# tnibler/local-features

Measured on AMD Instinct MI355X. Metric: MKD descriptors/sec (32x32 patch, 128-D), higher is better.
Workload: dtype f32 (f16x3 split MFMA pooling)

## Files before the change

### local-features_amd/csrc/mkd_describe.hip

```cpp
#include <hip/hip_runtime.h>
#include <stdint.h>

#include <type_traits>

#include "mkd_ablate.h"
#include "mkd_device.h"
#include "mkd_sample.h"

namespace lfmkd {


namespace {

typedef _Float16 f16x8 __attribute__((ext_vector_type(8)));
typedef unsigned int u32x4 __attribute__((ext_vector_type(4)));
typedef float f32x2 __attribute__((ext_vector_type(2)));
__device__ __forceinline__ f32x2 pk_fma(f32x2 a, f32x2 b, f32x2 c) { return __builtin_elementwise_fma(a, b, c); }
__device__ __forceinline__ f32x2 pk_set(float v) { return f32x2{v, v}; }

__device__ __host__ constexpr bool f16_family(int pool) { return pool == LF_POOL_F16X3 || pool == LF_POOL_F16_FP6; }

__device__ __host__ constexpr bool fold_form(int pool) { return pool != LF_POOL_F16_FP6; }
constexpr int kTiles = 21;
constexpr int kAccTiles = 21, kUnfAccTiles = 24;
// ... 5 lines not shown

constexpr float kB0 = 0.0096f, kB1 = 0.2054f, kB2 = 0.5699f;

__device__ __host__ constexpr int row_bytes(bool fold) { return lut_pieces(fold) * 1024; }
__device__ __host__ constexpr int ring_off(bool fold) { return 2 * row_bytes(fold); }
constexpr int kRowBytes = row_bytes(true), kRingOff = ring_off(true);
constexpr int kRingSlots = 6;
[[maybe_unused]] constexpr int kSrcPatches = 0, kSrcKeypoints = 1, kSrcKeypointsSplit = 2;
constexpr int kRingSlotsKp = 12;
constexpr int kLevelTableBytes = 5 * kMaxPyrLevels * 4;

__device__ __forceinline__ float lane_fetch(int byte_addr, float v) {
    return __int_as_float(__builtin_amdgcn_ds_bpermute(byte_addr, __float_as_int(v)));
}

__device__ __forceinline__ void lds_dma16(const void *gsrc, void *ldst) {
    __builtin_amdgcn_global_load_lds((const __attribute__((address_space(1))) void *)gsrc,
                                     (__attribute__((address_space(3))) void *)ldst, 16, 0, 0);
}
__device__ __forceinline__ void lds_dma16_sv(const unsigned char *uniform_base, unsigned lane_off, void *ldst) {
    asm("" : "+s"(uniform_base));
    asm volatile("" : "+v"(lane_off));
    lds_dma16(uniform_base + lane_off, ldst);
}

template <int W, bool FOLD, bool ODDV>
__device__ __forceinline__ void issue_lut_row(const unsigned char *__restrict__ lut_rows, int row,
                                              unsigned char *lds_row, int wave, int lane) {
    static_assert(!ODDV || FOLD, "the folded forms' tiles");
    constexpr int kPieces = ODDV ? lut_pieces(FOLD) - 8 : lut_pieces(FOLD);
    const unsigned lane16 = (unsigned)lane * 16u;
#pragma unroll
    for (int j = 0; j < (kPieces + W - 1) / W; ++j) {
        if (wave + W * j < kPieces) {
            const int i = wave + W * j, piece = ODDV ? i + 2 * (i >> 2) : i;
            const unsigned char *g = lut_rows + ((size_t)row * row_bytes(FOLD) + (size_t)piece * 1024);
            lds_dma16_sv(g, lane16, lds_row + piece * 1024);
        }
    }
}

constexpr int kWStepBytes = 16384;
__device__ __forceinline__ constexpr int wstage_slot(int step) { return step % 3 == 0 ? 0 : (step % 3 == 1 ? 32768 : 16384); }
static_assert(wstage_slot(0) + kWStepBytes <= row_bytes(true) && wstage_slot(10) >= row_bytes(false) &&
              wstage_slot(10) + kWStepBytes <= 2 * row_bytes(true), "both forms' row buffers");

template <int W>
__device__ __forceinline__ void issue_w_step(const unsigned char *__restrict__ wfrag, int step, unsigned char *lds,
                                             int wave, int lane) {
    const unsigned lane16 = (unsigned)lane * 16u;
    unsigned char *d = lds + wstage_slot(step);
#pragma unroll
    for (int j = 0; j < 16 / W; ++j) {
        const unsigned char *g = wfrag + ((size_t)step * kWStepBytes + (size_t)(wave + W * j) * 1024);
        lds_dma16_sv(g, lane16, d + (wave + W * j) * 1024);
    }
}

template <int N> __device__ __forceinline__ void wait_vmcnt() { asm volatile("s_waitcnt vmcnt(%0)" ::"n"(N) : "memory"); }

struct RawSrc { const unsigned char *base; unsigned lane_off; };
__device__ __forceinline__ void issue_raw_row(const RawSrc &src, int row, unsigned char *ring, int slot) {
    const int y = row < 0 ? 0 : (row > 31 ? 31 : row);
    const unsigned char *g = src.base + y * 128;
    lds_dma16_sv(g, src.lane_off, ring + slot * 2048);
    lds_dma16_sv(g + 64, src.lane_off, ring + slot * 2048 + 1024);
}

#pragma clang fp contract(off)

__device__ __forceinline__ float max3_tiny(float a, float b) {
    return __builtin_fmaxf(__builtin_fmaxf(a, b), 1e-30f);
}

template <int ANGLE>
__device__ __forceinline__ void gradient_direction(f32x2 gx, f32x2 gy, f32x2 r2, f32x2 &ct, f32x2 &st) {
    if (ANGLE == LF_ANGLE_EXACT || ANGLE == LF_ANGLE_EXACT_ZERO) {
        const f32x2 inv = {__builtin_amdgcn_rsqf(r2.x), __builtin_amdgcn_rsqf(r2.y)};
        const f32x2 c = gx * inv, s = -gy * inv;
        const bool z0 = ANGLE == LF_ANGLE_EXACT ? r2.x == 0.f : gx.x == 0.f;
        const bool z1 = ANGLE == LF_ANGLE_EXACT ? r2.y == 0.f : gx.y == 0.f;
        ct = f32x2{z0 ? 1.f : c.x, z1 ? 1.f : c.y};
        st = f32x2{z0 ? 0.f : s.x, z1 ? 0.f : s.y};
    } else {
        const float ax0 = fabsf(gx.x), ay0 = fabsf(gy.x), ax1 = fabsf(gx.y), ay1 = fabsf(gy.y);
        const bool sw0 = ax0 < ay0 && gx.x != 0.f, sw1 = ax1 < ay1 && gx.y != 0.f;
        const f32x2 mn = {__builtin_fminf(ax0, ay0), __builtin_fminf(ax1, ay1)};
        const f32x2 mx = {max3_tiny(ax0, ay0), max3_tiny(ax1, ay1)};
        const f32x2 a = mn * f32x2{__builtin_amdgcn_rcpf(mx.x), __builtin_amdgcn_rcpf(mx.y)};
        const f32x2 s = a * a;
        f32x2 p = pk_fma(s, pk_set(-0.0117212f), pk_set(0.05265332f));
        p = pk_fma(s, p, pk_set(-0.11643287f));
        p = pk_fma(s, p, pk_set(0.19354346f));
        p = pk_fma(s, p, pk_set(-0.33262347f));
        p = pk_fma(s, p, pk_set(0.99997726f));
        p = a * p;
        const f32x2 p2 = p * p;
// ... 150 lines not shown
    }
};

template <int POOL, int PART>
__device__ __forceinline__ void mma_part(const AFrag<POOL> &a, const BFrag &b, f32x4 &acc) {
    static_assert(POOL == LF_POOL_F32 || POOL == LF_POOL_F16X3, "the three-term / f32 forms");
    if constexpr (ablate::kNoMma && POOL == LF_POOL_F16X3) {
        asm volatile("" ::"v"(a.hi), "v"(a.lo), "v"(b.p0), "v"(b.p1));
        return;
    }
    if constexpr (POOL == LF_POOL_F32) {
        const f32x4 b0 = __builtin_bit_cast(f32x4, b.p0), b1 = __builtin_bit_cast(f32x4, b.p1);
        if (PART == 0) {
#pragma unroll
            for (int e = 0; e < 3; ++e) acc = __builtin_amdgcn_mfma_f32_16x16x4f32(b0[e], a.v[e], acc, 0, 0, 0);
        } else if (PART == 1) {
            acc = __builtin_amdgcn_mfma_f32_16x16x4f32(b0[3], a.v[3], acc, 0, 0, 0);
            acc = __builtin_amdgcn_mfma_f32_16x16x4f32(b1[0], a.v[4], acc, 0, 0, 0);
            acc = __builtin_amdgcn_mfma_f32_16x16x4f32(b1[1], a.v[5], acc, 0, 0, 0);
        } else {
            acc = __builtin_amdgcn_mfma_f32_16x16x4f32(b1[2], a.v[6], acc, 0, 0, 0);
            acc = __builtin_amdgcn_mfma_f32_16x16x4f32(b1[3], a.v[7], acc, 0, 0, 0);
        }
    } else {
        const f16x8 bh = __builtin_bit_cast(f16x8, b.p0), bl = __builtin_bit_cast(f16x8, b.p1);
        const f16x8 ah = __builtin_bit_cast(f16x8, a.hi), al = __builtin_bit_cast(f16x8, a.lo);
        if (PART == 0) acc = __builtin_amdgcn_mfma_f32_16x16x32_f16(bh, al, acc, 0, 0, 0);
        else if (PART == 1) acc = __builtin_amdgcn_mfma_f32_16x16x32_f16(bl, ah, acc, 0, 0, 0);
        else acc = __builtin_amdgcn_mfma_f32_16x16x32_f16(bh, ah, acc, 0, 0, 0);
    }
}

template <class SlotOfTap>
__device__ __forceinline__ void blur_row_impl(const unsigned char *ring_lane, SlotOfTap slot_of_tap, int addr_l, int addr_r,
                                              bool has_l, bool has_r, float (&out)[8], float &out_l, float &out_r) {
    if constexpr (ablate::kNoFrontEnd) {
        const int sl = slot_of_tap(0);
        const f32x4 a_ = *reinterpret_cast<const f32x4 *>(ring_lane + sl * 2048);
        const f32x4 b_ = *reinterpret_cast<const f32x4 *>(ring_lane + sl * 2048 + 256);
#pragma unroll
        for (int x = 0; x < 4; ++x) { out[x] = a_[x]; out[4 + x] = b_[x]; }
        out_l = out[0];
        out_r = out[7];
        return;
    }
    float vb[8];
    {
        const float kk[5] = {kB0, kB1, kB2, kB1, kB0};
        f32x2 v2[4];
#pragma unroll
        for (int i = 0; i < 5; ++i) {
            const int sl = slot_of_tap(i);
            const f32x4 lo = *reinterpret_cast<const f32x4 *>(ring_lane + sl * 2048);
            const f32x4 hi = *reinterpret_cast<const f32x4 *>(ring_lane + sl * 2048 + 256);
            const f32x2 r[4] = {{lo[0], lo[1]}, {lo[2], lo[3]}, {hi[0], hi[1]}, {hi[2], hi[3]}};
#pragma unroll
            for (int e = 0; e < 4; ++e) v2[e] = i == 0 ? pk_set(kk[0]) * r[e] : pk_fma(pk_set(kk[i]), r[e], v2[e]);
        }
#pragma unroll
        for (int e = 0; e < 4; ++e) { vb[2 * e] = v2[e].x; vb[2 * e + 1] = v2[e].y; }
    }
    float ext[12];
    const float l0 = lane_fetch(addr_l, vb[6]), l1 = lane_fetch(addr_l, vb[7]);
    const float r0 = lane_fetch(addr_r, vb[0]), r1 = lane_fetch(addr_r, vb[1]);
    ext[0] = has_l ? l0 : vb[0];
    ext[1] = has_l ? l1 : vb[0];
    ext[10] = has_r ? r0 : vb[7];
    ext[11] = has_r ? r1 : vb[7];
#pragma unroll
    for (int x = 0; x < 8; ++x) ext[2 + x] = vb[x];
#pragma unroll
    for (int x = 0; x < 8; ++x) {
        float s = ablate::kMulFirstTap ? kB0 * ext[x] : fmaf(kB0, ext[x], 0.0f);
        s = fmaf(kB1, ext[x + 1], s);
        s = fmaf(kB2, ext[x + 2], s);
        s = fmaf(kB1, ext[x + 3], s);
        s = fmaf(kB0, ext[x + 4], s);
        out[x] = s;
    }
    const float hl = lane_fetch(addr_l, out[7]), hr = lane_fetch(addr_r, out[0]);
    out_l = has_l ? hl : out[0];
    out_r = has_r ? hr : out[7];
}

template <class SlotOfTap>
__device__ __forceinline__ void blur_row_fold_impl(const unsigned char *ring_a, const unsigned char *ring_b, SlotOfTap slot_of_tap,
                                                   int addr_l, int addr_r, bool has_l, bool has_r, float (&out)[8],
                                                   float (&nb)[4]) {
    if constexpr (ablate::kNoFrontEnd) {
        const int sl = slot_of_tap(0);
        const f32x4 a_ = *reinterpret_cast<const f32x4 *>(ring_a + sl * 2048);
        const f32x4 b_ = *reinterpret_cast<const f32x4 *>(ring_b + sl * 2048);
#pragma unroll
        for (int x = 0; x < 4; ++x) { out[x] = a_[x]; out[4 + x] = b_[3 - x]; }
        nb[0] = out[0]; nb[1] = out[3]; nb[2] = out[7]; nb[3] = out[4];
        return;
    }
    float va[4], vb[4];
    {
        const float kk[5] = {kB0, kB1, kB2, kB1, kB0};
        f32x2 v2[4];
#pragma unroll
        for (int i = 0; i < 5; ++i) {
            const int sl = slot_of_tap(i);
            const f32x4 lo = *reinterpret_cast<const f32x4 *>(ring_a + sl * 2048);
            const f32x4 hi = *reinterpret_cast<const f32x4 *>(ring_b + sl * 2048);
            const f32x2 r[4] = {{lo[0], lo[1]}, {lo[2], lo[3]}, {hi[0], hi[1]}, {hi[2], hi[3]}};
#pragma unroll
            for (int e = 0; e < 4; ++e) v2[e] = i == 0 ? pk_set(kk[0]) * r[e] : pk_fma(pk_set(kk[i]), r[e], v2[e]);
        }
        va[0] = v2[0].x; va[1] = v2[0].y; va[2] = v2[1].x; va[3] = v2[1].y;
        vb[0] = v2[2].x; vb[1] = v2[2].y; vb[2] = v2[3].x; vb[3] = v2[3].y;
    }
    float ea[8], eb[8];
    {
        const float la0 = lane_fetch(addr_l, va[2]), la1 = lane_fetch(addr_l, va[3]);
        const float rb0 = lane_fetch(addr_l, vb[0]), rb1 = lane_fetch(addr_l, vb[1]);
        const float ra0 = lane_fetch(addr_r, va[0]), ra1 = lane_fetch(addr_r, va[1]);
        const float lb0 = lane_fetch(addr_r, vb[2]), lb1 = lane_fetch(addr_r, vb[3]);
        ea[0] = has_l ? la0 : va[0];
        ea[1] = has_l ? la1 : va[0];
        ea[6] = has_r ? ra0 : vb[0];
        ea[7] = has_r ? ra1 : vb[1];
        eb[0] = has_r ? lb0 : va[2];
        eb[1] = has_r ? lb1 : va[3];
        eb[6] = has_l ? rb0 : vb[3];
        eb[7] = has_l ? rb1 : vb[3];
    }
#pragma unroll
    for (int x = 0; x < 4; ++x) { ea[2 + x] = va[x]; eb[2 + x] = vb[x]; }
    float ob[4];
#pragma unroll
    for (int x = 0; x < 4; ++x) {
        float s = ablate::kMulFirstTap ? kB0 * ea[x] : fmaf(kB0, ea[x], 0.0f);
        s = fmaf(kB1, ea[x + 1], s);
        s = fmaf(kB2, ea[x + 2], s);
        s = fmaf(kB1, ea[x + 3], s);
        s = fmaf(kB0, ea[x + 4], s);
        out[x] = s;
        float t = ablate::kMulFirstTap ? kB0 * eb[x] : fmaf(kB0, eb[x], 0.0f);
        t = fmaf(kB1, eb[x + 1], t);
        t = fmaf(kB2, eb[x + 2], t);
        t = fmaf(kB1, eb[x + 3], t);
        t = fmaf(kB0, eb[x + 4], t);
        ob[x] = t;
    }
#pragma unroll
    for (int x = 0; x < 4; ++x) out[4 + x] = ob[3 - x];
    const float hal = lane_fetch(addr_l, out[3]), hbr = lane_fetch(addr_l, ob[0]);
    const float har = lane_fetch(addr_r, out[0]), hbl = lane_fetch(addr_r, ob[3]);
    nb[0] = has_l ? hal : out[0];
    nb[1] = has_r ? har : ob[0];
    nb[2] = has_r ? hbl : out[3];
    nb[3] = has_l ? hbr : ob[3];
}

__device__ __forceinline__ void fold_sum(const f32x2 (&s)[4], f32x2 &e0, f32x2 &e1) { e0 = s[0] + s[2]; e1 = s[1] + s[3]; }
__device__ __forceinline__ void fold_diff(const f32x2 (&s)[4], f32x2 &o0, f32x2 &o1) { o0 = s[0] - s[2]; o1 = s[1] - s[3]; }
__device__ __forceinline__ void fold_diff_rev(const f32x2 (&s)[4], f32x2 &o0, f32x2 &o1) { o0 = s[2] - s[0]; o1 = s[3] - s[1]; }

__device__ __forceinline__ void odd_cart_row(const f32x2 (&fx)[2], const f32x4 &gy, f32x2 h0, f32x2 h1, float (&oc)[3]) {
    const f32x2 r = pk_fma(fx[1], h1, fx[0] * h0);
    const float t = r.x + r.y;
#pragma unroll
    for (int b = 0; b < 3; ++b) oc[b] = __builtin_fmaf(gy[b], t, oc[b]);
}

__device__ __forceinline__ void rebuild_odd_cart(const float (&oc)[kOddCartSums][3], int lane, f32x4 (&acc)[kAccTiles]) {
    constexpr float kVm[4] = {0.37872374f, 0.51796234f, 0.46882015f, 0.39798096f};
#pragma unroll
    for (int s = 0; s < kOddCartSums; ++s) {
        const int k = (s + 1) / 2, t = s == 0 ? 2 : 3 + 6 * (k - 1) + 4 + ((s - 1) & 1);
        f32x4 d = {0.f, 0.f, 0.f, 0.f};
#pragma unroll
        for (int b = 0; b < 3; ++b)
            d = __builtin_amdgcn_mfma_f32_16x16x4f32((lane & 15) == b ? kVm[k] : 0.f, oc[s][b], d, 0, 0, 0);
        acc[t] = d;
    }
}

template <int POOL>
__device__ __forceinline__ void pool_harmonics(const f32x2 (&m)[4], const f32x2 (&c1)[4], const f32x2 (&s1)[4],
                                               const unsigned char *brow, BFrag &g, f32x4 (&acc)[kAccTiles],
                                               const f32x2 (&fx)[2], const f32x4 &gy, float (&oc)[kOddCartSums][3]) {
    f32x2 pk[4], qk[4], pp[4], qp[4], tc[4];
    AFrag<POOL> au, av;
#pragma unroll
    for (int e = 0; e < 4; ++e) { pk[e] = m[e] * c1[e]; qk[e] = m[e] * s1[e]; tc[e] = c1[e] + c1[e]; }
#pragma unroll
    for (int k = 0; k < 3; ++k) {
        {
            f32x2 u[4], v[4];
            fold_sum(pk, u[0], u[1]);
            fold_diff(qk, u[2], u[3]);
            fold_sum(qk, v[0], v[1]);
            fold_diff_rev(pk, v[2], v[3]);
            if constexpr (valu_odd_cart(POOL)) {
                odd_cart_row(fx, gy, u[2], u[3], oc[1 + 2 * k]);
                odd_cart_row(fx, gy, v[2], v[3], oc[2 + 2 * k]);
            }
            if constexpr (POOL == LF_POOL_F16X3) {
                AFrag<POOL>::set2(au, u, av, v);
// ... 539 lines not shown
    };
#pragma unroll 1
    for (int st = 0; st < sp.hi - sp.lo; st += 2) {
        step(st, ta, tb);
        step(st + 1, tb, ta);
    }
    asm volatile("s_waitcnt vmcnt(0) lgkmcnt(0)" ::: "memory");
    if (sp.consumer) {
#pragma unroll 1
        for (int e = 0; e < 12; ++e) __syncthreads();
    }
}

constexpr int kSplitSpinMax = 1 << 21;

}

template <int ANGLE, int POOL, int W, int SRC>
__global__ __launch_bounds__(SRC != kSrcPatches ? 128 * W : 64 * W) void mkd_pool(
    const float *__restrict__ patches, long n_host, const unsigned long long *__restrict__ n_dev,
    const unsigned char *__restrict__ lut_rows, const short *__restrict__ colmap, const unsigned char *__restrict__ wfrag,
    const float *__restrict__ bias, const float *__restrict__ odd_cart, float *__restrict__ out, float *__restrict__ raw_out,
    std::conditional_t<SRC != kSrcPatches, KpSource, int> ks, unsigned long long *__restrict__ clk) {
    constexpr bool kKp = SRC != kSrcPatches, kSplit = SRC == kSrcKeypointsSplit;
    static_assert(!kSplit || W == 2, "the row-split form is the narrow (2 + 2 wave) form");
    if (clk && blockIdx.x == 0 && threadIdx.x == 0) {
        clk[0] = __builtin_readcyclecounter();
        clk[1] = __builtin_amdgcn_s_memrealtime();
    }
    constexpr int kSlots = kKp ? kRingSlotsKp : kRingSlots;
    static_assert(!kKp || POOL == LF_POOL_F16X3, "keypoint mode pools in f16x3");
    constexpr int kMPool = POOL == LF_POOL_F16_FP6 ? LF_POOL_F16X3 : POOL;
    constexpr bool kFold = fold_form(POOL), kOddV = valu_odd_cart(POOL);
    static_assert(!kKp || (kFold && kOddV), "the producers write the folded forms' LDS map and request f16x3's LUT pieces");
    constexpr int kNAcc = acc_tiles(kFold), kRowB = row_bytes(kFold), kRingO = ring_off(kFold);
    __shared__ __attribute__((aligned(16))) unsigned char s_mem[kRingO + W * kSlots * 2048 +
                                                                (kKp ? kLevelTableBytes + kMaxPyrLevels * 8 : 0)];
    const long n = n_dev ? (long)*n_dev : n_host;
    const int lane = threadIdx.x & 63;
    const int wave = __builtin_amdgcn_readfirstlane(threadIdx.x >> 6);
    const int p = lane & 15, q = lane >> 4;
    const int addr_l = ((lane - 16) & 63) * 4, addr_r = ((lane + 16) & 63) * 4;
    const bool has_l = q > 0, has_r = q < 3;
    const long nbatch = (n + 16 * W - 1) / (16 * W);
    unsigned char *ring = s_mem + kRingO + wave * (kSlots * 2048);
    BatchWalk walk{(long)blockIdx.x, nbatch, (long)gridDim.x};
    [[maybe_unused]] RowSpan span{0, 32, 0, 32, 7, true};
    [[maybe_unused]] int role = 0, n_roles = 1;
    if constexpr (kKp) {
        if constexpr (kSplit) {
            n_roles = ks.split;
            const long id = blockIdx.x, grp = id / (8 * n_roles), in = id - grp * (8 * n_roles);
            role = (int)(in >> 3);
            const long b = grp * 8 + (in & 7);
            walk = BatchWalk{b, b < nbatch ? b + 1 : b, 1};
            span = row_span(role, n_roles);
        } else {
            walk = kp_batches(nbatch);
        }
        if (walk.cur >= walk.end) return;
        int *lv = reinterpret_cast<int *>(s_mem + kRingO + W * kSlots * 2048);
        long *lv_off = reinterpret_cast<long *>(lv + 5 * kMaxPyrLevels);
        if (threadIdx.x < kMaxPyrLevels) {
            const int l = threadIdx.x;
            int w_ = 0, h_ = 0, pi_ = 0, ap_ = 0;
            long of_ = 0;
// ... 4 lines not shown
            lv_off[l] = of_;
        }
        __syncthreads();
        const LevelTable lt{ks.pd.levels, lv, lv + kMaxPyrLevels, lv + 2 * kMaxPyrLevels, lv + 3 * kMaxPyrLevels};
        if (wave >= W) {
            if constexpr (kSplit) kp_produce_split<W>(ks, lt, lv_off, n, walk.cur, span, s_mem, lut_rows, wave - W, lane);
            else kp_produce<W>(ks, lt, lv_off, n, walk, s_mem, lut_rows, wave - W, lane);
            return;
        }

        if constexpr (ablate::kConsumerPrio >= 0) __builtin_amdgcn_s_setprio(ablate::kConsumerPrio);
    }
    const unsigned char *ring_lane = kFold ? ring + (q * 16 + p) * 16 : ring + (q >> 1) * 1024 + ((2 * (q & 1)) * 16 + p) * 16;
    [[maybe_unused]] const unsigned char *ring_mirror = ring + 1024 + ((3 - q) * 16 + p) * 16;

    long batch = walk.cur;
    if (batch >= walk.end) return;
    [[maybe_unused]] f32x2 oc_fx[2] = {pk_set(0.f), pk_set(0.f)};
    if constexpr (kOddV) {
        const f32x4 f = *reinterpret_cast<const f32x4 *>(odd_cart + 4 * q);
        oc_fx[0] = f32x2{f[0], f[1]};
        oc_fx[1] = f32x2{f[2], f[3]};
        asm volatile("" : "+v"(oc_fx[0]), "+v"(oc_fx[1]));
    }
    auto raw_src = [&](const float *pt, long b) {
        const long b0 = b * (16 * W) + wave * 16;
        const long wave0 = b0 < n ? b0 : n - 1;
        const long pidx = b0 + p < n ? b0 + p : n - 1;
        return RawSrc{reinterpret_cast<const unsigned char *>(pt + wave0 * 1024), (unsigned)(pidx - wave0) * 4096u + 16u * q};
    };
    {
        if constexpr (!kKp) {
            const RawSrc src = raw_src(patches, batch);
#pragma unroll
            for (int r = -2; r <= 3; ++r) issue_raw_row(src, r, ring, r + 2);
        }
        issue_lut_row<W, kFold, kOddV>(lut_rows, kSplit ? span.lo : 0, s_mem, wave, lane);
    }
    int slot0 = 0;
    unsigned par = 0;
    ablate::PhaseClock phase;
    phase.start();

    for (; batch < walk.end; batch += walk.step) {
        const unsigned char *wf = wfrag, *lr = lut_rows;
        const float *bs = bias, *pt = patches;
        float *o = out, *ro = raw_out;
        const short *cm = colmap;
        asm volatile("" : "+s"(wf), "+s"(bs), "+s"(lr), "+s"(o), "+s"(ro), "+s"(cm), "+s"(pt));
        const float *oc_tab = odd_cart;
        const long base = batch * (16 * W) + wave * 16;
        const bool more = batch + walk.step < walk.end;
        const RawSrc src = kKp ? RawSrc{nullptr, 0u} : raw_src(pt, batch);
        const RawSrc src_next = !kKp && more ? raw_src(pt, batch + walk.step) : src;

        f32x4 acc[kNAcc];
#pragma unroll
        for (int t = 0; t < kNAcc; ++t) acc[t] = f32x4{0.f, 0.f, 0.f, 0.f};
        [[maybe_unused]] float oc[kOddCartSums][3];
#pragma unroll
        for (int s = 0; s < kOddCartSums; ++s)
#pragma unroll
            for (int b = 0; b < 3; ++b) oc[s][b] = 0.f;
        float cur[8], prv[8], cur_nb[4] = {0.f, 0.f, 0.f, 0.f};
        int s0 = 1;

        auto patch_row = [&](auto kind, const int g) __attribute__((always_inline)) {
            constexpr bool kFirst = decltype(kind)::value == 0, kLast = decltype(kind)::value == 2;
            constexpr bool kFirstInner = decltype(kind)::value == 3;

            phase.mark(7);
            if constexpr (!ablate::kNoRowSync) {
                asm volatile("s_waitcnt vmcnt(0)" ::: "memory");
                __syncthreads();
            }
            phase.mark(0);
            const unsigned char *brow = s_mem + par * kRowB + lane * 16;
            if (f16_family(POOL) ? !kLast : (!kLast || more)) {
                if constexpr (!kKp) issue_lut_row<W, kFold, kOddV>(lr, (g + 1) & 31, s_mem + (par ^ 1) * kRowB, wave, lane);
            } else if (f16_family(POOL)) {
                issue_w_step<W>(wf, 0, s_mem, wave, lane);
            }
            par ^= 1;
            constexpr int kMTiles = kOddV ? 2 : 3;
            BFrag bm[kMTiles];
#pragma unroll
            for (int t = 0; t < kMTiles; ++t) bm[t] = load_b(brow, t);
            [[maybe_unused]] f32x4 oc_gy = {0.f, 0.f, 0.f, 0.f};
            if constexpr (kOddV) oc_gy = *reinterpret_cast<const f32x4 *>(oc_tab + 16 + 4 * g);

            if constexpr (!kKp)
                if (!kFirst && !kLast && g <= 29) issue_raw_row(src, g + 4, ring, s0 == 0 ? kRingSlots - 1 : s0 - 1);
            auto kp_slot = [&](int y, int i) {
                int r_ = y - 2 + i;
                r_ = r_ < 0 ? 0 : (r_ > 31 ? 31 : r_);
                return (slot0 + r_) % kRingSlotsKp;
            };
            auto blur = [&](auto tap, float (&o)[8], float (&o_nb)[4]) __attribute__((always_inline)) {
                if constexpr (kFold) blur_row_fold_impl(ring_lane, ring_mirror, tap, addr_l, addr_r, has_l, has_r, o, o_nb);
                else blur_row_impl(ring_lane, tap, addr_l, addr_r, has_l, has_r, o, o_nb[0], o_nb[1]);
            };
            auto ring_tap = [](int first) {
                return [first](int i) { const int sl = first + i; return sl >= kRingSlots ? sl - kRingSlots : sl; };
            };
            if (kFirst) {
                if constexpr (kKp) blur([&](int i) { return kp_slot(0, i); }, cur, cur_nb);
                else blur(ring_tap(0), cur, cur_nb);
#pragma unroll
                for (int x = 0; x < 8; ++x) prv[x] = cur[x];
            }
            if constexpr (kFirstInner) {
                float edge[4];
                blur([&](int i) { return kp_slot(g - 1, i); }, prv, edge);
                blur([&](int i) { return kp_slot(g, i); }, cur, cur_nb);
            }
            float nxt[8], nxt_nb[4] = {0.f, 0.f, 0.f, 0.f};
            if (!kLast) {
                if constexpr (kKp) blur([&](int i) { return kp_slot(g + 1, i); }, nxt, nxt_nb);
                else blur(ring_tap(s0), nxt, nxt_nb);
            } else {
#pragma unroll
                for (int x = 0; x < 8; ++x) nxt[x] = cur[x];
#pragma unroll
                for (int x = 0; x < 4; ++x) nxt_nb[x] = cur_nb[x];
            }
            asm volatile("" ::: "memory");
            if constexpr (!kKp) {
                if (kFirst) {
                    issue_raw_row(src, g + 4, ring, s0 == 0 ? kRingSlots - 1 : s0 - 1);
                } else if (kLast && more) {
#pragma unroll
                    for (int r = -2; r <= 3; ++r) issue_raw_row(src_next, r, ring, r + 2);
                }
            }
            s0 = s0 == kRingSlots - 1 ? 0 : s0 + 1;
            phase.mark(1);

            f32x2 m[4], c1[4], s1[4];
            {
                f32x2 gx[4], gy[4], r2n[4];
#pragma unroll
                for (int e = 0; e < 4; ++e) {
                    const int x = 2 * e;
                    f32x2 left, right;
                    if constexpr (kFold) {
                        left = e == 0 ? f32x2{cur_nb[0], cur[0]} : e == 1 ? f32x2{cur[1], cur[2]}
                               : e == 2 ? f32x2{cur[5], cur[6]} : f32x2{cur[7], cur_nb[2]};
                        right = e == 0 ? f32x2{cur[1], cur[2]} : e == 1 ? f32x2{cur[3], cur_nb[1]}
                                : e == 2 ? f32x2{cur_nb[3], cur[4]} : f32x2{cur[5], cur[6]};
                    } else {
                        left = f32x2{x == 0 ? cur_nb[0] : cur[x - 1], cur[x]};
                        right = f32x2{cur[x + 1], x == 6 ? cur_nb[1] : cur[x + 2]};
                    }
                    gx[e] = (left - right) + pk_set(0.0f);
                    gy[e] = f32x2{nxt[x], nxt[x + 1]} - f32x2{prv[x], prv[x + 1]};
                    r2n[e] = pk_fma(gy[e], gy[e], gx[e] * gx[e]);
                    const f32x2 r2 = r2n[e] + pk_set(1e-8f);
                    m[e] = f32x2{__builtin_amdgcn_sqrtf(__builtin_amdgcn_sqrtf(r2.x)),
                                 __builtin_amdgcn_sqrtf(__builtin_amdgcn_sqrtf(r2.y))};
                }
                if constexpr (ablate::kNoFrontEnd) {
#pragma unroll
                    for (int e = 0; e < 4; ++e) { c1[e] = gx[e]; s1[e] = gy[e]; }
                } else {
                    gradient_direction4<ANGLE>(gx, gy, r2n, c1, s1);
                }
            }
#pragma unroll
            for (int x = 0; x < 8; ++x) {
                prv[x] = cur[x];
                cur[x] = nxt[x];
            }
#pragma unroll
            for (int x = 0; x < 4; ++x) cur_nb[x] = nxt_nb[x];
            phase.mark(2);

            BFrag gfrag = load_b(brow, 3);
            {
                AFrag<kMPool> am;
                if constexpr (kFold) {
                    f32x2 mf[4];
                    fold_sum(m, mf[0], mf[1]);
                    fold_diff(m, mf[2], mf[3]);
                    if constexpr (kOddV) odd_cart_row(oc_fx, oc_gy, mf[2], mf[3], oc[0]);
                    am.set(mf);
                } else {
                    am.set(m);
                }
#pragma unroll
                for (int t = 0; t < kMTiles; ++t) mma_part<kMPool, 0>(am, bm[t], acc[t]);
#pragma unroll
                for (int t = 0; t < kMTiles; ++t) mma_part<kMPool, 1>(am, bm[t], acc[t]);
#pragma unroll
                for (int t = 0; t < kMTiles; ++t) mma_part<kMPool, 2>(am, bm[t], acc[t]);
            }
            phase.mark(3);
            if constexpr (POOL == LF_POOL_F16_FP6) pool_harmonics_fp6(m, c1, s1, brow, gfrag, acc);
            else pool_harmonics<POOL>(m, c1, s1, brow, gfrag, acc, oc_fx, oc_gy, oc);
            phase.mark(4);
            phase.mark(5);
        };
        if constexpr (kSplit) {
            if (span.lo == 0) patch_row(std::integral_constant<int, 0>(), 0);
            else patch_row(std::integral_constant<int, 3>(), span.lo);
#pragma unroll 1
            for (int g = span.lo + 1; g < span.hi - 1; ++g) patch_row(std::integral_constant<int, 1>(), g);
            if (span.consumer) patch_row(std::integral_constant<int, 2>(), span.hi - 1);
            else patch_row(std::integral_constant<int, 1>(), span.hi - 1);
            if constexpr (kOddV) rebuild_odd_cart(oc, lane, acc);
            unsigned *cnt = ks.xchg_cnt + batch * W + wave;
            typedef unsigned long long u64;
            if (!span.consumer) {
                u64 *dst = reinterpret_cast<u64 *>(ks.xchg + ((((long)batch * (n_roles - 1) + role) * W + wave) * kAccTiles) * 256) + lane;
#pragma unroll
                for (int t = 0; t < kAccTiles; ++t) {
                    const u64 v0 = ((u64)__float_as_uint(acc[t][1]) << 32) | __float_as_uint(acc[t][0]);
                    const u64 v1 = ((u64)__float_as_uint(acc[t][3]) << 32) | __float_as_uint(acc[t][2]);
                    __hip_atomic_store(dst + t * 128, v0, __ATOMIC_RELAXED, __HIP_MEMORY_SCOPE_AGENT);
                    __hip_atomic_store(dst + t * 128 + 64, v1, __ATOMIC_RELAXED, __HIP_MEMORY_SCOPE_AGENT);
                }
                asm volatile("s_waitcnt vmcnt(0)" ::: "memory");
                if (lane == 0) __hip_atomic_fetch_add(cnt, 1u, __ATOMIC_RELAXED, __HIP_MEMORY_SCOPE_AGENT);
                if (clk && blockIdx.x == 0 && threadIdx.x == 0) {
                    clk[2] = __builtin_readcyclecounter();
                    clk[3] = __builtin_amdgcn_s_memrealtime();
                }
                return;
            }
            int polls = 0;
            while (__hip_atomic_load(cnt, __ATOMIC_RELAXED, __HIP_MEMORY_SCOPE_AGENT) != (unsigned)(n_roles - 1) &&
                   polls < kSplitSpinMax) {
                __builtin_amdgcn_s_sleep(1);
                ++polls;
            }
            asm volatile("" ::: "memory");
            if (polls >= kSplitSpinMax && lane == 0) atomicAdd(ks.xchg_cnt - 1, 1u);
#pragma unroll 1
            for (int r = 0; r + 1 < n_roles; ++r) {
                const u64 *srcp = reinterpret_cast<const u64 *>(ks.xchg + ((((long)batch * (n_roles - 1) + r) * W + wave) * kAccTiles) * 256) + lane;
                u64 v[2 * kAccTiles];
#pragma unroll
                for (int t = 0; t < 2 * kAccTiles; ++t)
                    v[t] = __hip_atomic_load(srcp + t * 64, __ATOMIC_RELAXED, __HIP_MEMORY_SCOPE_AGENT);
                __builtin_amdgcn_sched_barrier(0);
#pragma unroll
                for (int t = 0; t < kAccTiles; ++t)
                    acc[t] += f32x4{__uint_as_float((unsigned)v[2 * t]), __uint_as_float((unsigned)(v[2 * t] >> 32)),
                                    __uint_as_float((unsigned)v[2 * t + 1]), __uint_as_float((unsigned)(v[2 * t + 1] >> 32))};
            }
            if (lane == 0) __hip_atomic_store(cnt, 0u, __ATOMIC_RELAXED, __HIP_MEMORY_SCOPE_AGENT);
            asm volatile("s_waitcnt vmcnt(0)" ::: "memory");
        } else {
            patch_row(std::integral_constant<int, 0>(), 0);
#pragma unroll 1
            for (int g = 1; g < ablate::kRows - 1; ++g) patch_row(std::integral_constant<int, 1>(), g);
            patch_row(std::integral_constant<int, 2>(), ablate::kRows - 1);
            if constexpr (kOddV) rebuild_odd_cart(oc, lane, acc);
        }
        if constexpr (ablate::kNoEpilogue) {
            f32x4 sum = acc[0];
            for (int t = 1; t < kNAcc; ++t) sum += acc[t];
            if (base + p < n) *reinterpret_cast<f32x4 *>(out + (base + p) * 128 + 4 * q) = sum;
            if (f16_family(POOL)) {
                __syncthreads();
                if (more) issue_lut_row<W, kFold, kOddV>(lr, 0, s_mem, wave, lane);
            }
        } else {
            finish_descriptors<POOL, W>(acc, lane, wave, base + p < n, base + p, cm, wf, bs, o, ro, s_mem, lr, more);
        }
        phase.mark(6);
        if constexpr (kKp) slot0 = (slot0 + 8) % kRingSlotsKp;
    }
    phase.dump(out, wave, lane);
    if (clk && blockIdx.x == 0 && threadIdx.x == 0) {
        clk[2] = __builtin_readcyclecounter();
        clk[3] = __builtin_amdgcn_s_memrealtime();
    }
}

#ifndef LF_DESCRIBE_KP
void launch_describe(const float *patches, long n, const unsigned long long *n_dev, const DeviceConsts &dc,
                     int angle_mode, int pool_mode, float *out, float *raw_out, int num_cus, hipStream_t stream, int waves,
                     unsigned long long *clk) {
    if (n <= 0) return;
    const bool small = ablate::kForceFourWaves || waves == 4 || (waves != 8 && n <= 64L * num_cus);
    const long nbatch = small ? (n + 63) / 64 : (n + 127) / 128;
    const unsigned grid = (unsigned)(nbatch < num_cus ? nbatch : num_cus);
    const bool f16 = f16_family(pool_mode);
    const unsigned char *lut = pool_mode == LF_POOL_F16_FP6 ? reinterpret_cast<const unsigned char *>(dc.pool_b_fp6)
                               : f16                        ? reinterpret_cast<const unsigned char *>(dc.pool_b_f16)
                                                            : reinterpret_cast<const unsigned char *>(dc.pool_b_f32);
    const bool unfolded = !fold_form(pool_mode);
    const unsigned char *wf = unfolded ? reinterpret_cast<const unsigned char *>(dc.white_a_f16_unfolded)
                              : f16    ? reinterpret_cast<const unsigned char *>(dc.white_a_f16)
                                       : reinterpret_cast<const unsigned char *>(dc.white_a_f32);
    const short *colmap = unfolded ? dc.colmap_unfolded : dc.colmap;
#define LF_LAUNCH_W(A, P, WV)                                                                                          \
    hipLaunchKernelGGL((mkd_pool<A, P, WV, kSrcPatches>), dim3(grid), dim3(64 * WV), 0, stream, patches, n, n_dev, lut, \
                       colmap, wf, dc.white_bias, dc.odd_cart, out, raw_out, 0, clk)
#define LF_LAUNCH(A, P)            \
    do {                           \
// ... 81 lines not shown
```

Baseline: 305.6 million.

## Blur patch rows in pairs sharing ring loads and restructure raw-row prefetch

New measurement: 317.8 million (median of 6 runs). 4.0% higher.

```diff
diff --git a/local-features_amd/csrc/mkd_describe.hip b/local-features_amd/csrc/mkd_describe.hip
--- a/local-features_amd/csrc/mkd_describe.hip
+++ b/local-features_amd/csrc/mkd_describe.hip
@@ -61,7 +61,7 @@
     const unsigned lane16 = (unsigned)lane * 16u;
 #pragma unroll
     for (int j = 0; j < (kPieces + W - 1) / W; ++j) {
-        if (wave + W * j < kPieces) {
+        if (kPieces % W == 0 || wave + W * j < kPieces) {
             const int i = wave + W * j, piece = ODDV ? i + 2 * (i >> 2) : i;
             const unsigned char *g = lut_rows + ((size_t)row * row_bytes(FOLD) + (size_t)piece * 1024);
             lds_dma16_sv(g, lane16, lds_row + piece * 1024);
@@ -89,9 +89,9 @@
 template <int N> __device__ __forceinline__ void wait_vmcnt() { asm volatile("s_waitcnt vmcnt(%0)" ::"n"(N) : "memory"); }
 
 struct RawSrc { const unsigned char *base; unsigned lane_off; };
+__device__ __forceinline__ constexpr int clamp_row(int row) { return row < 0 ? 0 : (row > 31 ? 31 : row); }
 __device__ __forceinline__ void issue_raw_row(const RawSrc &src, int row, unsigned char *ring, int slot) {
-    const int y = row < 0 ? 0 : (row > 31 ? 31 : row);
-    const unsigned char *g = src.base + y * 128;
+    const unsigned char *g = src.base + row * 128;
     lds_dma16_sv(g, src.lane_off, ring + slot * 2048);
     lds_dma16_sv(g + 64, src.lane_off, ring + slot * 2048 + 1024);
 }
@@ -308,33 +308,74 @@
 }
 
 template <class SlotOfTap>
-__device__ __forceinline__ void blur_row_impl(const unsigned char *ring_lane, SlotOfTap slot_of_tap, int addr_l, int addr_r,
-                                              bool has_l, bool has_r, float (&out)[8], float &out_l, float &out_r) {
+__device__ __forceinline__ void vblur_row(const unsigned char *ring_a, const unsigned char *ring_b, SlotOfTap slot_of_tap,
+                                          float (&v)[8]) {
     if constexpr (ablate::kNoFrontEnd) {
         const int sl = slot_of_tap(0);
-        const f32x4 a_ = *reinterpret_cast<const f32x4 *>(ring_lane + sl * 2048);
-        const f32x4 b_ = *reinterpret_cast<const f32x4 *>(ring_lane + sl * 2048 + 256);
-#pragma unroll
-        for (int x = 0; x < 4; ++x) { out[x] = a_[x]; out[4 + x] = b_[x]; }
+        const f32x4 a_ = *reinterpret_cast<const f32x4 *>(ring_a + sl * 2048);
+        const f32x4 b_ = *reinterpret_cast<const f32x4 *>(ring_b + sl * 2048);
+#pragma unroll
+        for (int x = 0; x < 4; ++x) { v[x] = a_[x]; v[4 + x] = b_[x]; }
+        return;
+    }
+    const float kk[5] = {kB0, kB1, kB2, kB1, kB0};
+    f32x2 v2[4];
+#pragma unroll
+    for (int i = 0; i < 5; ++i) {
+        const int sl = slot_of_tap(i);
+        const f32x4 lo = *reinterpret_cast<const f32x4 *>(ring_a + sl * 2048);
+        const f32x4 hi = *reinterpret_cast<const f32x4 *>(ring_b + sl * 2048);
+        const f32x2 r[4] = {{lo[0], lo[1]}, {lo[2], lo[3]}, {hi[0], hi[1]}, {hi[2], hi[3]}};
+#pragma unroll
+        for (int e = 0; e < 4; ++e) v2[e] = i == 0 ? pk_set(kk[0]) * r[e] : pk_fma(pk_set(kk[i]), r[e], v2[e]);
+    }
+#pragma unroll
+    for (int e = 0; e < 4; ++e) { v[2 * e] = v2[e].x; v[2 * e + 1] = v2[e].y; }
+}
+
+template <int NR, class SlotOfRow, class TapA, class TapB>
+__device__ __forceinline__ void vblur_pair(const unsigned char *ring_a, const unsigned char *ring_b, SlotOfRow slot_of_row,
+                                           TapA tap_a, TapB tap_b, float (&va)[8], float (&vb)[8]) {
+    f32x2 r[NR][4];
+#pragma unroll
+    for (int j = 0; j < NR; ++j) {
+        const int sl = slot_of_row(j);
+        const f32x4 lo = *reinterpret_cast<const f32x4 *>(ring_a + sl * 2048);
+        const f32x4 hi = *reinterpret_cast<const f32x4 *>(ring_b + sl * 2048);
+        r[j][0] = f32x2{lo[0], lo[1]}; r[j][1] = f32x2{lo[2], lo[3]};
+        r[j][2] = f32x2{hi[0], hi[1]}; r[j][3] = f32x2{hi[2], hi[3]};
+    }
+    f32x2 a2[4], b2[4];
+    if constexpr (ablate::kNoFrontEnd) {
+#pragma unroll
+        for (int e = 0; e < 4; ++e) { a2[e] = r[tap_a(0)][e]; b2[e] = r[tap_b(0)][e]; }
+    } else {
+        const float kk[5] = {kB0, kB1, kB2, kB1, kB0};
+#pragma unroll
+        for (int i = 0; i < 5; ++i) {
+            const int ja = tap_a(i), jb = tap_b(i);
+#pragma unroll
+            for (int e = 0; e < 4; ++e) {
+                a2[e] = i == 0 ? pk_set(kk[0]) * r[ja][e] : pk_fma(pk_set(kk[i]), r[ja][e], a2[e]);
+                b2[e] = i == 0 ? pk_set(kk[0]) * r[jb][e] : pk_fma(pk_set(kk[i]), r[jb][e], b2[e]);
+            }
+        }
+    }
+#pragma unroll
+    for (int e = 0; e < 4; ++e) {
+        va[2 * e] = a2[e].x; va[2 * e + 1] = a2[e].y;
+        vb[2 * e] = b2[e].x; vb[2 * e + 1] = b2[e].y;
+    }
+}
+
+__device__ __forceinline__ void hblur_row(const float (&vb)[8], int addr_l, int addr_r, bool has_l, bool has_r, float (&out)[8],
+                                          float &out_l, float &out_r) {
+    if constexpr (ablate::kNoFrontEnd) {
+#pragma unroll
+        for (int x = 0; x < 8; ++x) out[x] = vb[x];
         out_l = out[0];
         out_r = out[7];
         return;
-    }
-    float vb[8];
-    {
-        const float kk[5] = {kB0, kB1, kB2, kB1, kB0};
-        f32x2 v2[4];
-#pragma unroll
-        for (int i = 0; i < 5; ++i) {
-            const int sl = slot_of_tap(i);
-            const f32x4 lo = *reinterpret_cast<const f32x4 *>(ring_lane + sl * 2048);
-            const f32x4 hi = *reinterpret_cast<const f32x4 *>(ring_lane + sl * 2048 + 256);
-            const f32x2 r[4] = {{lo[0], lo[1]}, {lo[2], lo[3]}, {hi[0], hi[1]}, {hi[2], hi[3]}};
-#pragma unroll
-            for (int e = 0; e < 4; ++e) v2[e] = i == 0 ? pk_set(kk[0]) * r[e] : pk_fma(pk_set(kk[i]), r[e], v2[e]);
-        }
-#pragma unroll
-        for (int e = 0; e < 4; ++e) { vb[2 * e] = v2[e].x; vb[2 * e + 1] = v2[e].y; }
     }
     float ext[12];
     const float l0 = lane_fetch(addr_l, vb[6]), l1 = lane_fetch(addr_l, vb[7]);
@@ -360,34 +401,22 @@
 }
 
 template <class SlotOfTap>
-__device__ __forceinline__ void blur_row_fold_impl(const unsigned char *ring_a, const unsigned char *ring_b, SlotOfTap slot_of_tap,
-                                                   int addr_l, int addr_r, bool has_l, bool has_r, float (&out)[8],
-                                                   float (&nb)[4]) {
+__device__ __forceinline__ void blur_row_impl(const unsigned char *ring_lane, SlotOfTap slot_of_tap, int addr_l, int addr_r,
+                                              bool has_l, bool has_r, float (&out)[8], float &out_l, float &out_r) {
+    float vb[8];
+    vblur_row(ring_lane, ring_lane + 256, slot_of_tap, vb);
+    hblur_row(vb, addr_l, addr_r, has_l, has_r, out, out_l, out_r);
+}
+
+__device__ __forceinline__ void hblur_row_fold(const float (&v)[8], int addr_l, int addr_r, bool has_l, bool has_r,
+                                               float (&out)[8], float (&nb)[4]) {
     if constexpr (ablate::kNoFrontEnd) {
-        const int sl = slot_of_tap(0);
-        const f32x4 a_ = *reinterpret_cast<const f32x4 *>(ring_a + sl * 2048);
-        const f32x4 b_ = *reinterpret_cast<const f32x4 *>(ring_b + sl * 2048);
-#pragma unroll
-        for (int x = 0; x < 4; ++x) { out[x] = a_[x]; out[4 + x] = b_[3 - x]; }
+#pragma unroll
+        for (int x = 0; x < 4; ++x) { out[x] = v[x]; out[4 + x] = v[7 - x]; }
         nb[0] = out[0]; nb[1] = out[3]; nb[2] = out[7]; nb[3] = out[4];
         return;
     }
-    float va[4], vb[4];
-    {
-        const float kk[5] = {kB0, kB1, kB2, kB1, kB0};
-        f32x2 v2[4];
-#pragma unroll
-        for (int i = 0; i < 5; ++i) {
-            const int sl = slot_of_tap(i);
-            const f32x4 lo = *reinterpret_cast<const f32x4 *>(ring_a + sl * 2048);
-            const f32x4 hi = *reinterpret_cast<const f32x4 *>(ring_b + sl * 2048);
-            const f32x2 r[4] = {{lo[0], lo[1]}, {lo[2], lo[3]}, {hi[0], hi[1]}, {hi[2], hi[3]}};
-#pragma unroll
-            for (int e = 0; e < 4; ++e) v2[e] = i == 0 ? pk_set(kk[0]) * r[e] : pk_fma(pk_set(kk[i]), r[e], v2[e]);
-        }
-        va[0] = v2[0].x; va[1] = v2[0].y; va[2] = v2[1].x; va[3] = v2[1].y;
-        vb[0] = v2[2].x; vb[1] = v2[2].y; vb[2] = v2[3].x; vb[3] = v2[3].y;
-    }
+    const float va[4] = {v[0], v[1], v[2], v[3]}, vb[4] = {v[4], v[5], v[6], v[7]};
     float ea[8], eb[8];
     {
         const float la0 = lane_fetch(addr_l, va[2]), la1 = lane_fetch(addr_l, va[3]);
@@ -431,6 +460,15 @@
     nb[3] = has_l ? hbr : ob[3];
 }
 
+template <class SlotOfTap>
+__device__ __forceinline__ void blur_row_fold_impl(const unsigned char *ring_a, const unsigned char *ring_b, SlotOfTap slot_of_tap,
+                                                   int addr_l, int addr_r, bool has_l, bool has_r, float (&out)[8],
+                                                   float (&nb)[4]) {
+    float v[8];
+    vblur_row(ring_a, ring_b, slot_of_tap, v);
+    hblur_row_fold(v, addr_l, addr_r, has_l, has_r, out, nb);
+}
+
 __device__ __forceinline__ void fold_sum(const f32x2 (&s)[4], f32x2 &e0, f32x2 &e1) { e0 = s[0] + s[2]; e1 = s[1] + s[3]; }
 __device__ __forceinline__ void fold_diff(const f32x2 (&s)[4], f32x2 &o0, f32x2 &o1) { o0 = s[0] - s[2]; o1 = s[1] - s[3]; }
 __device__ __forceinline__ void fold_diff_rev(const f32x2 (&s)[4], f32x2 &o0, f32x2 &o1) { o0 = s[2] - s[0]; o1 = s[3] - s[1]; }
@@ -444,6 +482,7 @@
 
 __device__ __forceinline__ void rebuild_odd_cart(const float (&oc)[kOddCartSums][3], int lane, f32x4 (&acc)[kAccTiles]) {
     constexpr float kVm[4] = {0.37872374f, 0.51796234f, 0.46882015f, 0.39798096f};
+    asm volatile("" : "+v"(lane));
 #pragma unroll
     for (int s = 0; s < kOddCartSums; ++s) {
         const int k = (s + 1) / 2, t = s == 0 ? 2 : 3 + 6 * (k - 1) + 4 + ((s - 1) & 1);
@@ -1049,6 +1088,7 @@
     static_assert(!kKp || POOL == LF_POOL_F16X3, "keypoint mode pools in f16x3");
     constexpr int kMPool = POOL == LF_POOL_F16_FP6 ? LF_POOL_F16X3 : POOL;
     constexpr bool kFold = fold_form(POOL), kOddV = valu_odd_cart(POOL);
+    constexpr bool kPairs = SRC == kSrcPatches && POOL == LF_POOL_F16X3;
     static_assert(!kKp || (kFold && kOddV), "the producers write the folded forms' LDS map and request f16x3's LUT pieces");
     constexpr int kNAcc = acc_tiles(kFold), kRowB = row_bytes(kFold), kRingO = ring_off(kFold);
     __shared__ __attribute__((aligned(16))) unsigned char s_mem[kRingO + W * kSlots * 2048 +
@@ -1119,8 +1159,13 @@
     {
         if constexpr (!kKp) {
             const RawSrc src = raw_src(patches, batch);
-#pragma unroll
-            for (int r = -2; r <= 3; ++r) issue_raw_row(src, r, ring, r + 2);
+            if constexpr (kPairs) {
+#pragma unroll
+                for (int r = 0; r < kRingSlots; ++r) issue_raw_row(src, r, ring, r);
+            } else {
+#pragma unroll
+                for (int r = -2; r <= 3; ++r) issue_raw_row(src, clamp_row(r), ring, r + 2);
+            }
         }
         issue_lut_row<W, kFold, kOddV>(lut_rows, kSplit ? span.lo : 0, s_mem, wave, lane);
     }
@@ -1150,11 +1195,17 @@
 #pragma unroll
             for (int b = 0; b < 3; ++b) oc[s][b] = 0.f;
         float cur[8], prv[8], cur_nb[4] = {0.f, 0.f, 0.f, 0.f};
-        int s0 = 1;
-
-        auto patch_row = [&](auto kind, const int g) __attribute__((always_inline)) {
+        [[maybe_unused]] float vnext[8];
+        [[maybe_unused]] bool last_six = false;
+        [[maybe_unused]] int s0 = 1;
+
+        auto patch_row = [&](auto kind, const int g, auto pos) __attribute__((always_inline)) {
             constexpr bool kFirst = decltype(kind)::value == 0, kLast = decltype(kind)::value == 2;
             constexpr bool kFirstInner = decltype(kind)::value == 3;
+            constexpr int kPos = decltype(pos)::value;
+            constexpr bool kPairFirst = kPos >= 0 && (kPos & 1) == 0, kPairSecond = kPos >= 0 && (kPos & 1) == 1;
+            constexpr int kSlot0 = kPos >= 0 ? (kPos & ~1) : 0;
+            static_assert(kPairs ? (kFirst || kLast) == (kPos < 0) : kPos < 0, "the pair forms' rows 1..30 go in pairs");
 
             phase.mark(7);
             if constexpr (!ablate::kNoRowSync) {
@@ -1176,51 +1227,94 @@
             [[maybe_unused]] f32x4 oc_gy = {0.f, 0.f, 0.f, 0.f};
             if constexpr (kOddV) oc_gy = *reinterpret_cast<const f32x4 *>(oc_tab + 16 + 4 * g);
 
-            if constexpr (!kKp)
-                if (!kFirst && !kLast && g <= 29) issue_raw_row(src, g + 4, ring, s0 == 0 ? kRingSlots - 1 : s0 - 1);
-            auto kp_slot = [&](int y, int i) {
-                int r_ = y - 2 + i;
-                r_ = r_ < 0 ? 0 : (r_ > 31 ? 31 : r_);
-                return (slot0 + r_) % kRingSlotsKp;
-            };
-            auto blur = [&](auto tap, float (&o)[8], float (&o_nb)[4]) __attribute__((always_inline)) {
-                if constexpr (kFold) blur_row_fold_impl(ring_lane, ring_mirror, tap, addr_l, addr_r, has_l, has_r, o, o_nb);
-                else blur_row_impl(ring_lane, tap, addr_l, addr_r, has_l, has_r, o, o_nb[0], o_nb[1]);
-            };
-            auto ring_tap = [](int first) {
-                return [first](int i) { const int sl = first + i; return sl >= kRingSlots ? sl - kRingSlots : sl; };
-            };
-            if (kFirst) {
-                if constexpr (kKp) blur([&](int i) { return kp_slot(0, i); }, cur, cur_nb);
-                else blur(ring_tap(0), cur, cur_nb);
-#pragma unroll
-                for (int x = 0; x < 8; ++x) prv[x] = cur[x];
-            }
-            if constexpr (kFirstInner) {
-                float edge[4];
-                blur([&](int i) { return kp_slot(g - 1, i); }, prv, edge);
-                blur([&](int i) { return kp_slot(g, i); }, cur, cur_nb);
-            }
+            if constexpr (!kKp && !kPairs)
+                if (!kFirst && !kLast && g <= 29) issue_raw_row(src, clamp_row(g + 4), ring, s0 == 0 ? kRingSlots - 1 : s0 - 1);
             float nxt[8], nxt_nb[4] = {0.f, 0.f, 0.f, 0.f};
-            if (!kLast) {
-                if constexpr (kKp) blur([&](int i) { return kp_slot(g + 1, i); }, nxt, nxt_nb);
-                else blur(ring_tap(s0), nxt, nxt_nb);
+            if constexpr (!kPairs) {
+                auto kp_slot = [&](int y, int i) {
+                    int r_ = y - 2 + i;
+                    r_ = r_ < 0 ? 0 : (r_ > 31 ? 31 : r_);
+                    return (slot0 + r_) % kRingSlotsKp;
+                };
+                auto blur = [&](auto tap, float (&o)[8], float (&o_nb)[4]) __attribute__((always_inline)) {
+                    if constexpr (kFold) blur_row_fold_impl(ring_lane, ring_mirror, tap, addr_l, addr_r, has_l, has_r, o, o_nb);
+                    else blur_row_impl(ring_lane, tap, addr_l, addr_r, has_l, has_r, o, o_nb[0], o_nb[1]);
+                };
+                auto ring_tap = [](int first) {
+                    return [first](int i) { const int sl = first + i; return sl >= kRingSlots ? sl - kRingSlots : sl; };
+                };
+                if (kFirst) {
+                    if constexpr (kKp) blur([&](int i) { return kp_slot(0, i); }, cur, cur_nb);
+                    else blur(ring_tap(0), cur, cur_nb);
+#pragma unroll
+                    for (int x = 0; x < 8; ++x) prv[x] = cur[x];
+                }
+                if constexpr (kFirstInner) {
+                    float edge[4];
+                    blur([&](int i) { return kp_slot(g - 1, i); }, prv, edge);
+                    blur([&](int i) { return kp_slot(g, i); }, cur, cur_nb);
+                }
+                if (!kLast) {
+                    if constexpr (kKp) blur([&](int i) { return kp_slot(g + 1, i); }, nxt, nxt_nb);
+                    else blur(ring_tap(s0), nxt, nxt_nb);
+                }
             } else {
+                const unsigned char *ring_b = kFold ? ring_mirror : ring_lane + 256;
+                auto hblur = [&](const float (&v)[8], float (&o)[8], float (&o_nb)[4]) __attribute__((always_inline)) {
+                    if constexpr (kFold) hblur_row_fold(v, addr_l, addr_r, has_l, has_r, o, o_nb);
+                    else hblur_row(v, addr_l, addr_r, has_l, has_r, o, o_nb[0], o_nb[1]);
+                };
+                auto slot = [](int j) { return (kSlot0 + j) % kRingSlots; };
+                if constexpr (kFirst) {
+                    float v0[8];
+                    vblur_pair<4>(ring_lane, ring_b, slot, [](int i) { return i < 2 ? 0 : i - 2; },
+                                  [](int i) { return i < 1 ? 0 : i - 1; }, v0, vnext);
+                    hblur(v0, cur, cur_nb);
+#pragma unroll
+                    for (int x = 0; x < 8; ++x) prv[x] = cur[x];
+                    hblur(vnext, nxt, nxt_nb);
+                } else if constexpr (kPairFirst) {
+                    float v1[8];
+                    if (kPos == 4 && last_six)
+                        vblur_pair<4>(ring_lane, ring_b, slot, [](int i) { return i < 3 ? i : 3; },
+                                      [](int i) { return i < 2 ? i + 1 : 3; }, v1, vnext);
+                    else
+                        vblur_pair<6>(ring_lane, ring_b, slot, [](int i) { return i; }, [](int i) { return i + 1; }, v1, vnext);
+                    asm volatile("s_waitcnt lgkmcnt(0)" ::: "memory");
+                    if (!last_six || kPos == 0) {
+                        issue_raw_row(src, g + 5, ring, kSlot0);
+                        issue_raw_row(src, g + 6, ring, kSlot0 + 1);
+                    } else if (more) {
+                        if constexpr (kPos == 2) {
+                            issue_raw_row(src_next, 2, ring, 2);
+                            issue_raw_row(src_next, 3, ring, 3);
+                        } else {
+#pragma unroll
+                            for (int r = 0; r < kRingSlots; ++r)
+                                if (r != 2 && r != 3) issue_raw_row(src_next, r, ring, r);
+                        }
+                    }
+                    hblur(v1, nxt, nxt_nb);
+                } else if constexpr (kPairSecond) {
+                    hblur(vnext, nxt, nxt_nb);
+                }
+            }
+            if (kLast) {
 #pragma unroll
                 for (int x = 0; x < 8; ++x) nxt[x] = cur[x];
 #pragma unroll
                 for (int x = 0; x < 4; ++x) nxt_nb[x] = cur_nb[x];
             }
             asm volatile("" ::: "memory");
-            if constexpr (!kKp) {
+            if constexpr (!kKp && !kPairs) {
                 if (kFirst) {
                     issue_raw_row(src, g + 4, ring, s0 == 0 ? kRingSlots - 1 : s0 - 1);
                 } else if (kLast && more) {
 #pragma unroll
-                    for (int r = -2; r <= 3; ++r) issue_raw_row(src_next, r, ring, r + 2);
+                    for (int r = -2; r <= 3; ++r) issue_raw_row(src_next, clamp_row(r), ring, r + 2);
                 }
-            }
-            s0 = s0 == kRingSlots - 1 ? 0 : s0 + 1;
+                s0 = s0 == kRingSlots - 1 ? 0 : s0 + 1;
+            }
             phase.mark(1);
 
             f32x2 m[4], c1[4], s1[4];
@@ -1285,15 +1379,19 @@
             if constexpr (POOL == LF_POOL_F16_FP6) pool_harmonics_fp6(m, c1, s1, brow, gfrag, acc);
             else pool_harmonics<POOL>(m, c1, s1, brow, gfrag, acc, oc_fx, oc_gy, oc);
             phase.mark(4);
+            if constexpr (kPairs)
+#pragma unroll
+                for (int s = 0; s < kOddCartSums; ++s) asm volatile("" : "+v"(oc[s][0]), "+v"(oc[s][1]), "+v"(oc[s][2]));
             phase.mark(5);
         };
+        constexpr std::integral_constant<int, -1> kOwnBody{};
         if constexpr (kSplit) {
-            if (span.lo == 0) patch_row(std::integral_constant<int, 0>(), 0);
-            else patch_row(std::integral_constant<int, 3>(), span.lo);
+            if (span.lo == 0) patch_row(std::integral_constant<int, 0>(), 0, kOwnBody);
+            else patch_row(std::integral_constant<int, 3>(), span.lo, kOwnBody);
 #pragma unroll 1
-            for (int g = span.lo + 1; g < span.hi - 1; ++g) patch_row(std::integral_constant<int, 1>(), g);
-            if (span.consumer) patch_row(std::integral_constant<int, 2>(), span.hi - 1);
-            else patch_row(std::integral_constant<int, 1>(), span.hi - 1);
+            for (int g = span.lo + 1; g < span.hi - 1; ++g) patch_row(std::integral_constant<int, 1>(), g, kOwnBody);
+            if (span.consumer) patch_row(std::integral_constant<int, 2>(), span.hi - 1, kOwnBody);
+            else patch_row(std::integral_constant<int, 1>(), span.hi - 1, kOwnBody);
             if constexpr (kOddV) rebuild_odd_cart(oc, lane, acc);
             unsigned *cnt = ks.xchg_cnt + batch * W + wave;
             typedef unsigned long long u64;
@@ -1338,10 +1436,25 @@
             if (lane == 0) __hip_atomic_store(cnt, 0u, __ATOMIC_RELAXED, __HIP_MEMORY_SCOPE_AGENT);
             asm volatile("s_waitcnt vmcnt(0)" ::: "memory");
         } else {
-            patch_row(std::integral_constant<int, 0>(), 0);
+            patch_row(std::integral_constant<int, 0>(), 0, kOwnBody);
+            if constexpr (!kPairs) {
 #pragma unroll 1
-            for (int g = 1; g < ablate::kRows - 1; ++g) patch_row(std::integral_constant<int, 1>(), g);
-            patch_row(std::integral_constant<int, 2>(), ablate::kRows - 1);
+                for (int g = 1; g < ablate::kRows - 1; ++g) patch_row(std::integral_constant<int, 1>(), g, kOwnBody);
+                patch_row(std::integral_constant<int, 2>(), ablate::kRows - 1, kOwnBody);
+            } else {
+                static_assert(ablate::kRows == 32, "LF_ABLATE_ROWS: the pair forms walk whole patches only");
+#pragma unroll 1
+                for (int g = 1; g < 31; g += 6) {
+                    last_six = g == 25;
+                    patch_row(std::integral_constant<int, 1>(), g, std::integral_constant<int, 0>());
+                    patch_row(std::integral_constant<int, 1>(), g + 1, std::integral_constant<int, 1>());
+                    patch_row(std::integral_constant<int, 1>(), g + 2, std::integral_constant<int, 2>());
+                    patch_row(std::integral_constant<int, 1>(), g + 3, std::integral_constant<int, 3>());
+                    patch_row(std::integral_constant<int, 1>(), g + 4, std::integral_constant<int, 4>());
+                    patch_row(std::integral_constant<int, 1>(), g + 5, std::integral_constant<int, 5>());
+                }
+                patch_row(std::integral_constant<int, 2>(), 31, kOwnBody);
+            }
             if constexpr (kOddV) rebuild_odd_cart(oc, lane, acc);
         }
         if constexpr (ablate::kNoEpilogue) {
@@ -1353,7 +1466,10 @@
                 if (more) issue_lut_row<W, kFold, kOddV>(lr, 0, s_mem, wave, lane);
             }
         } else {
-            finish_descriptors<POOL, W>(acc, lane, wave, base + p < n, base + p, cm, wf, bs, o, ro, s_mem, lr, more);
+            int lane_e = lane;
+            if constexpr (kPairs) asm volatile("" : "+v"(lane_e));
+            const long patch_e = base + (lane_e & 15);
+            finish_descriptors<POOL, W>(acc, lane_e, wave, patch_e < n, patch_e, cm, wf, bs, o, ro, s_mem, lr, more);
         }
         phase.mark(6);
         if constexpr (kKp) slot0 = (slot0 + 8) % kRingSlotsKp;
```
